# danshapero/sigma

Measured on AMD Instinct MI355X. Metric: SpMV GB/s (achieved HBM) + CG iters/sec on 5-pt Laplacian, N=1e7, higher is better.
Workload: dtype f64; 1 GPU; 5-point 2D Poisson CSR, 3162x3162 rows per GPU (rank 0: n=9998244, nnz=49978572), fp64 SpMV y=A*x; rows_per_gpu=9998244, nnz_per_gpu=49978572, parallelism=row-partition x1, matrix_resident_bytes_per_gpu=479920788, reference_layout_bytes_per_gpu=639735844, full=False

## Files before the change

### sigma_amd/__init__.py

```python
from __future__ import annotations

import ctypes as C
import os

import numpy as np

_HERE = os.path.dirname(os.path.abspath(__file__))
LIB_PATH = os.path.join(_HERE, "libsigma_hip.so")

SGM_HOST, SGM_DEVICE = 0, 1
FMT_CSR, FMT_ELL = 1, 2

_lib = None


class SigmaError(RuntimeError):

    def __init__(self, code, msg):
        super().__init__(f"[sigma_hip status {code}] {msg}")
        self.code = code


def build(force=False):
    import subprocess
# ... 221 lines not shown
        _ck(lib().sgm_graph_greedy_color_order(self._h, p.ctypes.data_as(C.c_void_p), ptrs.ctypes.data_as(C.c_void_p),
                                               C.c_int32(len(ptrs)), C.byref(nc)))
        return p, ptrs[:nc.value + 1].copy(), nc.value

    def left_permute(self, p):
        pp, w, _k = _arg(p, np.int32)
        _ck(lib().sgm_mat_left_permute(self._h, pp, C.c_int(w)))

    def right_permute(self, p):
        pp, w, _k = _arg(p, np.int32)
        _ck(lib().sgm_mat_right_permute(self._h, pp, C.c_int(w)))

    def set_option(self, name, value):
        if hasattr(self, "_build"):
            self._build()
        _ck(lib().sgm_mat_set_option(self._h, name.encode(), C.c_int(int(value))))
        return self

    @property
    def kernel(self):
        buf = C.create_string_buffer(64)
        _ck(lib().sgm_mat_kernel(self._h, buf, C.c_int(64)))
        return buf.value.decode()

    def set_solver(self, solver):
        self.solver = solver
        solver.setup(self)

    def set_preconditioner(self, pc):
        self.pc = pc
        pc.setup(self)

    def solve(self, x, b):
        if self.solver is None:
            raise SigmaError(1, "A%solve: no solver set (linear_operator_interface.f90:213-233)")
        return self.solver.solve(self, x, b, self.pc)

    def get(self, name, dtype):
        need = C.c_size_t(0)
        _ck(lib().sgm_mat_get(self._h, name.encode(), None, C.c_size_t(0), C.byref(need)))
        out = np.zeros(need.value // np.dtype(dtype).itemsize, dtype)
        _ck(lib().sgm_mat_get(self._h, name.encode(), C.c_void_p(out.ctypes.data), C.c_size_t(out.nbytes), None))
        return out

    def _triples(self, i, j, z=None):
        if not (_is_torch(i) or _is_torch(j) or (z is not None and _is_torch(z))):
# ... 971 lines not shown
```

### sigma_amd/csrc/sgm_internal.hpp

```cpp
#pragma once
#include <hip/hip_runtime.h>

#include <cstdarg>
#include <cstdint>
#include <cstdio>
#include <cstring>
#include <string>
#include <atomic>
#include <type_traits>
#include <utility>
#include <vector>

#include "../../include/sigma_hip.h"

namespace sgm {

extern std::string g_err;
int fail(int code, const char *fmt, ...);

#define SGM_HIP(call)                                                              \
    do {                                                                           \
        hipError_t e__ = (call);                                                   \
        if (e__ != hipSuccess)                                                     \
            return sgm::fail(SGM_ERR_HIP, "%s:%d: %s -> %s", __FILE__, __LINE__,   \
// ... 119 lines not shown
    int32_t recv_count = 0;
};

struct SliceSched { int32_t *tab = nullptr; int32_t lo = 0, hi = 0, grid = 0, iters = 0, band = 0; };

struct Part {
    MatOptions opt = g_opt.mat;
    int32_t n = 0;
    int32_t ncol_own = 0;
    int32_t n_halo = 0;
    int32_t int_lo = 0, int_hi = 0;
    int64_t nnz = 0;
    int64_t row_begin = 0;
    int32_t *rowptr = nullptr;
    int32_t *col = nullptr;
    double *val = nullptr;
    uint8_t *code = nullptr;
    int32_t *dict = nullptr;
    int32_t ndict = 0;
    int32_t dict_reach = 0;
    int32_t max_row = 0;
    double *sval = nullptr;
    uint32_t *scode = nullptr;
    int32_t *scol = nullptr;
    uint8_t *sbcode = nullptr;
    bool lean = false;
    double *sl_val = nullptr;
    int32_t *sl_col = nullptr;
    uint16_t *sl_perm = nullptr;
    int64_t *sl_off = nullptr;
    int64_t sl_total = 0;
    int32_t *sl_win0 = nullptr;
    int32_t sl_gs = 1;
    int32_t sl_span = 0;
    int32_t sw = 0;
    int32_t sched_period = 0;
    mutable SliceSched sched[3];
    mutable int nsched = 0;
    const int32_t *run_sched = nullptr;
    int32_t run_iters = 0;
    int32_t max_d = 0;
    int32_t *ecol = nullptr;
    double *eval = nullptr;
    int32_t *edeg = nullptr;
    uint8_t *ecode = nullptr;
    int32_t emdp = 0;
// ... 279 lines not shown
```

### sigma_amd/csrc/sgm_layouts.hip

```cpp
#include "sgm_spmv_select.hpp"

namespace sgm {

__global__ void k_dec1(int32_t *a, int64_t n)
{
    int64_t i = (int64_t)blockIdx.x * blockDim.x + threadIdx.x;
    const int64_t stride = (int64_t)gridDim.x * blockDim.x;
    for (; i < n; i += stride) a[i] -= 1;
}

__global__ void k_check_ptr1(const int32_t *__restrict__ ptr1, int64_t n, int64_t nnz, unsigned long long *bad)
{
    int64_t i = (int64_t)blockIdx.x * blockDim.x + threadIdx.x;
    const int64_t stride = (int64_t)gridDim.x * blockDim.x;
    for (; i <= n; i += stride) {
        const int32_t a = ptr1[i];
        bool ok = true;
        if (i == 0) ok = a == 1;
        if (i < n) ok = ok && ptr1[i + 1] >= a;
        else ok = ok && (int64_t)a - 1 == nnz;
        if (!ok) atomicMin(bad, (unsigned long long)i);
    }
}

// ... 144 lines not shown
    const int64_t nsl = ((int64_t)n + kSlRows - 1) / kSlRows;
    for (int64_t sl = blockIdx.x; sl < nsl; sl += gridDim.x)
        for (int r = threadIdx.x; r < kSlRows; r += blockDim.x) {
            const int64_t row = sl * kSlRows + r;
            int32_t k = 0, ke = 0;
            if (row < n) { k = rowptr[row]; ke = rowptr[row + 1]; }
            double *dst = sval + sl * (int64_t)W * kSlRows + r;
            for (int u = 0; u < W; ++u) dst[(int64_t)u * kSlRows] = k + u < ke ? val[k + u] : 0.0;
        }
}

__global__ __launch_bounds__(256) void k_sl_pack_ell(int32_t n, int32_t W, int32_t max_d, const double *__restrict__ eval,
                                                     double *__restrict__ sval)
{
    const int64_t nsl = ((int64_t)n + kSlRows - 1) / kSlRows;
    for (int64_t sl = blockIdx.x; sl < nsl; sl += gridDim.x)
        for (int r = threadIdx.x; r < kSlRows; r += blockDim.x) {
            const int64_t row = sl * kSlRows + r;
            double *dst = sval + sl * (int64_t)W * kSlRows + r;
            for (int u = 0; u < W; ++u) dst[(int64_t)u * kSlRows] = (row < n && u < max_d) ? eval[(int64_t)u * n + row] : 0.0;
        }
}

__global__ __launch_bounds__(256) void k_sl_unpack(int32_t n, int32_t W, const int32_t *__restrict__ rowptr, const uint32_t *__restrict__ scode,
                                                   const int32_t *__restrict__ dict, const double *__restrict__ sval,
                                                   int32_t *__restrict__ col, double *__restrict__ val, uint8_t *__restrict__ code)
{
    __shared__ int32_t dl[16];
    if (threadIdx.x < 16) dl[threadIdx.x] = dict[threadIdx.x];
    __syncthreads();
    for (int32_t i = blockIdx.x * blockDim.x + threadIdx.x; i < n; i += gridDim.x * blockDim.x) {
        const uint32_t cw = scode[i];
        int32_t k = rowptr[i];
        const double *src = sval + ((int64_t)(i >> 9) * W) * kSlRows + (i & (kSlRows - 1));
        for (int u = 0; u < W; ++u) {
            const uint32_t c = (cw >> (4 * u)) & 15u;
            if (c == 15u) break;
            if (col) col[k] = i + dl[c];
            if (val) val[k] = src[(int64_t)u * kSlRows];
            if (code) code[k] = (uint8_t)c;
            ++k;
        }
    }
}
__global__ __launch_bounds__(256) void k_sell_unpack(int32_t n, const int32_t *__restrict__ rowptr, const int64_t *__restrict__ off,
                                                     const uint16_t *__restrict__ perm, const int32_t *__restrict__ scol,
// ... 65 lines not shown
    (void)hipStreamSynchronize(g_rt.stream);
    dfree(p.val); dfree(p.col); dfree(p.code);
    p.val = nullptr; p.col = nullptr; p.code = nullptr;
}

int pack_sliced(Part &p)
{
    if (p.sl_val && p.n > 0) {
        const int64_t nch = (((int64_t)p.n + kSlRows - 1) / kSlRows) * (kSlRows / kSellChunk);
        hipLaunchKernelGGL(k_sell_fill, dim3((unsigned)std::min<int64_t>((nch + 3) / 4, 65536)), dim3(256), 0, g_rt.stream, p.n,
                           (const int32_t *)p.rowptr, (const int32_t *)nullptr, (const double *)p.val, (const int64_t *)p.sl_off,
                           (const uint16_t *)p.sl_perm, (int32_t *)nullptr, p.sl_val);
        SGM_HIP(hipGetLastError());
    }
    if ((!p.scode && !p.scol && !p.sbcode) || p.n == 0) return SGM_OK;
    const int64_t nsl = ((int64_t)p.n + kSlRows - 1) / kSlRows;
    if (p.ecol)
        hipLaunchKernelGGL(k_sl_pack_ell, dim3((unsigned)std::min<int64_t>(nsl, 65536)), dim3(256), 0, g_rt.stream, p.n, p.sw,
                           p.max_d, (const double *)p.eval, p.sval);
    else
        hipLaunchKernelGGL(k_sl_pack, dim3((unsigned)std::min<int64_t>(nsl, 65536)), dim3(256), 0, g_rt.stream, p.n, p.sw,
                           (const int32_t *)p.rowptr, (const double *)p.val, p.sval);
    SGM_HIP(hipGetLastError());
    return SGM_OK;
}

__global__ void k_fill32(int64_t n, int32_t *a, int32_t v)
{
    int64_t i = (int64_t)blockIdx.x * blockDim.x + threadIdx.x;
    const int64_t stride = (int64_t)gridDim.x * blockDim.x;
    for (; i < n; i += stride) a[i] = v;
}

constexpr int kDictSlots = 1024;
constexpr int32_t kDictEmpty = INT32_MIN;
__global__ __launch_bounds__(256) void k_dict_collect(int32_t n, const int32_t *__restrict__ rowptr, const int32_t *__restrict__ col,
                                                      int32_t *table, int *count, int *max_row)
{
    constexpr int kLocal = 512;
    __shared__ int32_t ltab[kLocal];
    __shared__ int lcount;
    for (int t = threadIdx.x; t < kLocal; t += 256) ltab[t] = kDictEmpty;
    if (threadIdx.x == 0) lcount = 0;
    __syncthreads();
    int mr = 0;
    int32_t mine[8];
#pragma unroll
// ... 465 lines not shown
    q.opt.csr_offset_dict = 0; q.opt.csr_sliced = 0; q.opt.csr_sell = 0; q.opt.csr_lean = 0; q.opt.slice_sched = 0;
    q.n = p.n; q.ncol_own = p.ncol_own; q.n_halo = 0; q.nnz = p.nnz; q.max_row = p.max_row;
    hipStream_t st = g_rt.stream;
    int rc = dalloc(&q.rowptr, (size_t)p.n + 1);
    if (rc == SGM_OK) rc = dalloc(&q.col, (size_t)p.nnz + 4);
    if (rc == SGM_OK) rc = dalloc(&q.val, (size_t)p.nnz + 2);
    if (rc != SGM_OK) { sgm_mat_destroy(C); return rc; }
    (void)hipMemcpyAsync(q.rowptr, p.rowptr, ((size_t)p.n + 1) * 4, hipMemcpyDeviceToDevice, st);
    (void)hipMemsetAsync(q.col + p.nnz, 0, 16, st);
    (void)hipMemsetAsync(q.val + p.nnz, 0, 16, st);
    if (p.nnz) {
        (void)hipMemcpyAsync(q.col, p.col, (size_t)p.nnz * 4, hipMemcpyDeviceToDevice, st);
        (void)hipMemcpyAsync(q.val, p.val, (size_t)p.nnz * 8, hipMemcpyDeviceToDevice, st);
    }
    if (hipStreamSynchronize(st) != hipSuccess || hipGetLastError() != hipSuccess) { sgm_mat_destroy(C); return fail(SGM_ERR_HIP, "clone_csr_plain: copy failed"); }
    *out = C;
    return SGM_OK;
}

int rebuild_csr_formats(Part &p)
{
    SGM_TRY(csr_need_arrays(p));
    p.lean = false;
    dfree(p.code); dfree(p.dict); dfree(p.sval); dfree(p.scode); dfree(p.scol); dfree(p.sbcode);
    p.code = nullptr; p.dict = nullptr; p.sval = nullptr; p.scode = nullptr; p.scol = nullptr; p.sbcode = nullptr;
    free_sell(p);
    free_ell_colblock(p);
    p.ndict = 0; p.dict_reach = 0; p.sw = 0; p.max_row = 0; p.sched_period = 0;
    free_slice_sched(p);
    return build_offset_dict(p, nullptr, nullptr);
}
int rebuild_ell_formats(Part &p)
{
    dfree(p.ecode); dfree(p.dict); dfree(p.sval); dfree(p.scode);
    p.ecode = nullptr; p.dict = nullptr; p.dict_reach = 0; p.emdp = 0; p.sval = nullptr; p.scode = nullptr; p.sw = 0; p.sched_period = 0;
    free_slice_sched(p);
    SGM_TRY(build_ell_offset_dict(p));
    SGM_TRY(build_ell_colblock(p));
    return refresh_ell_colblock_values(p);
}
int sgm_invalidate_transpose(sgm_mat A)
{
    if (A->T) { sgm_mat_destroy(A->T); A->T = nullptr; }
    dfree(A->tperm);
    A->tperm = nullptr;
    A->t_stale = true;
    return SGM_OK;
}

void free_part(Part &p)
{
    dfree(p.rowptr); dfree(p.col); dfree(p.val); dfree(p.code); dfree(p.dict); dfree(p.sval); dfree(p.scode); dfree(p.scol); dfree(p.sbcode); dfree(p.ecol); dfree(p.eval); dfree(p.edeg); dfree(p.ecode); dfree(p.xext);
    for (auto &nb : p.nbrs) { dfree(nb.send_idx); dfree(nb.send_buf); }
    free_slice_sched(p);
    free_ell_colblock(p);
    free_sell(p);
    p = Part();
}

}
```

### sigma_amd/csrc/sgm_mat.hip

```cpp
#include "sgm_spmv_select.hpp"
#include "sgm_krylov.hpp"

namespace sgm {

int stage_in(Staged &s, const double *v, int64_t n, int where, bool copy)
{
    if (where == SGM_DEVICE && (reinterpret_cast<uintptr_t>(v) & 15) == 0) {
        s.dev = const_cast<double *>(v);
        return SGM_OK;
    }
    SGM_TRY(dalloc(&s.dev, (size_t)n));
    s.owned = true;
    if (copy)
        SGM_HIP(hipMemcpyAsync(s.dev, v, (size_t)n * 8,
                               where == SGM_HOST ? hipMemcpyHostToDevice : hipMemcpyDeviceToDevice,
                               g_rt.stream));
    return SGM_OK;
}
int stage_out(const Staged &s, double *v, int64_t n, int where)
{
    if (!s.owned) return SGM_OK;
    SGM_HIP(hipMemcpyAsync(v, s.dev, (size_t)n * 8,
                           where == SGM_HOST ? hipMemcpyDeviceToHost : hipMemcpyDeviceToDevice,
                           g_rt.stream));
// ... 521 lines not shown
    A->parts.resize(1);
    A->parts[0].n = (int32_t)nloc_r;
    A->parts[0].ncol_own = (int32_t)nloc_c;
    int64_t g = (nloc_r + 4 * kBlock - 1) / (4 * kBlock);
    A->parts[0].dot_grid_override = (int)std::max<int64_t>(1, std::min<int64_t>(g, 2048));
    *out = A;
    return SGM_OK;
}

int sgm_mat_matvec_t(sgm_mat A, const double *x, double *y, int where)
{
    return matvec_t_impl(A, x, y, where, false);
}

int sgm_mat_matvec_t_add(sgm_mat A, const double *x, double *y, int where)
{
    return matvec_t_impl(A, x, y, where, true);
}

int sgm_mat_get(sgm_mat A, const char *name, void *out, size_t bytes, size_t *needed)
{
    SGM_TRY(require_init());
    if (!A || !name) return fail(SGM_ERR_BAD_ARG, "sgm_mat_get: null argument");
    if (A->distributed() || A->fmt == SGM_FMT_COMPOSITE)
        return fail(SGM_ERR_UNSUPPORTED, "sgm_mat_get: leaf single-GPU matrices only");
    const Part &p = A->parts[0];
    const std::string nm(name);
    std::vector<int32_t> vi;
    std::vector<double> vd;
    std::vector<int64_t> vq;
    const bool ell = A->fmt == SGM_FMT_ELL;
    if (!ell && (nm == "node" || nm == "val")) SGM_TRY(csr_need_arrays(p));
    struct Release { const Part &p; bool on; ~Release() { if (on) csr_release_arrays(p); } } rel{p, !ell};
    SGM_HIP(hipStreamSynchronize(g_rt.stream));
    if (!ell && nm == "ptr") {
        vi.resize((size_t)p.n + 1);
        SGM_HIP(hipMemcpy(vi.data(), p.rowptr, vi.size() * 4, hipMemcpyDeviceToHost));
        for (auto &v : vi) v += 1;
    } else if (!ell && nm == "node") {
        vi.resize((size_t)p.nnz);
        if (p.nnz) SGM_HIP(hipMemcpy(vi.data(), p.col, vi.size() * 4, hipMemcpyDeviceToHost));
        for (auto &v : vi) v += 1;
    } else if (!ell && nm == "val") {
        vd.resize((size_t)p.nnz);
        if (p.nnz) SGM_HIP(hipMemcpy(vd.data(), p.val, vd.size() * 8, hipMemcpyDeviceToHost));
    } else if (ell && nm == "max_d") {
// ... 68 lines not shown
extern "C" {

int sgm_mat_kernel(sgm_mat A, char *buf, int len)
{
    if (!A || !buf || len < 1) return fail(SGM_ERR_BAD_ARG, "sgm_mat_kernel: bad argument");
    char name[64];
    if (A->fmt == SGM_FMT_COMPOSITE) snprintf(name, sizeof name, "composite");
    else part_kernel_name(A->parts[0], A->fmt, name, sizeof name);
    snprintf(buf, (size_t)len, "%s", name);
    return SGM_OK;
}

static int64_t part_resident_bytes(const Part &p)
{
    int64_t b = 0;
    const int64_t nsl = ((int64_t)p.n + kSlRows - 1) / kSlRows;
    if (p.rowptr) b += 4 * ((int64_t)p.n + 1);
    if (p.col) b += 4 * (p.nnz + 4);
    if (p.val) b += 8 * (p.nnz + 2);
    if (p.code) b += p.nnz + 16;
    if (p.dict) b += 4 * 256;
    if (p.sval) b += 8 * nsl * kSlRows * p.sw;
    if (p.scode) b += 4 * nsl * kSlRows;
    if (p.scol) b += 4 * nsl * kSlRows * p.sw;
    if (p.sbcode) b += nsl * kSlRows * ((p.sw + 7) / 8 * 8);
    if (p.sl_val) b += 12 * p.sl_total + 2 * nsl * kSlRows + 8 * (nsl * (kSlRows / kSellChunk) + 1);
    if (p.ecol) b += 4 * (int64_t)p.n * p.max_d;
    if (p.eval) b += 8 * (int64_t)p.n * p.max_d;
    if (p.edeg) b += 4 * (int64_t)p.n;
    if (p.ecode) b += (int64_t)p.n * p.emdp;
    if (p.xext) b += 8 * p.xlen();
    b += ell_colblock_resident_bytes(p);
    for (const auto &nb : p.nbrs) b += (int64_t)nb.send_count * (nb.send_buf ? 12 : 4);
    return b;
}
static int64_t part_matvec_bytes(const sgm_mat_s *A, const Part &p)
{
    const int64_t nsl = ((int64_t)p.n + kSlRows - 1) / kSlRows;
    int64_t m;
    if (A->fmt == SGM_FMT_ELL) {
        if (use_ell_colblock(p)) return ell_colblock_matvec_bytes(p);
        if (use_sliced_ell(p)) m = nsl * kSlRows * (8 * (int64_t)p.sw + 4);
        else if (p.ecode && p.opt.ell_offset_dict) m = (int64_t)p.n * (8 * (int64_t)p.max_d + p.emdp);
        else m = 12 * (int64_t)p.n * p.max_d;
    } else if (use_ell_colblock(p)) return ell_colblock_matvec_bytes(p);
    else if (use_sliced(p)) m = nsl * kSlRows * (8 * (int64_t)p.sw + 4);
    else if (use_slicedb(p)) m = nsl * kSlRows * (8 * (int64_t)p.sw + (p.sw + 7) / 8 * 8);
    else if (use_sliced32(p)) m = nsl * kSlRows * 12 * (int64_t)p.sw;
    else if (use_sell(p)) {
        m = 12 * p.sl_total + 2 * nsl * kSlRows + 8 * nsl * (kSlRows / kSellChunk);
        if (p.sl_win0 && p.opt.csr_xwindow)
            return m + ((nsl + p.sl_gs - 1) / p.sl_gs) * (8 * (int64_t)p.sl_span + 4) + 8 * (int64_t)p.n;
    }
    else if (use_offset_dict(p)) m = 9 * p.nnz + 4 * ((int64_t)p.n + 1);
    else m = 12 * p.nnz + 4 * ((int64_t)p.n + 1);
    return m + 8 * p.xlen() + 8 * (int64_t)p.n;
}

int sgm_mat_footprint(sgm_mat A, int64_t *resident_bytes, int64_t *matvec_bytes)
{
    if (!A) return fail(SGM_ERR_BAD_ARG, "sgm_mat_footprint: null matrix");
    int64_t res = 0, mv = 0;
    if (A->fmt == SGM_FMT_COMPOSITE) {
        for (sgm_mat C : A->blocks) {
            if (!C) continue;
            int64_t r = 0, m = 0;
            SGM_TRY(sgm_mat_footprint(C, &r, &m));
            mv += m + 8 * (int64_t)C->nrow;
        }
// ... 23 lines not shown
```

### sigma_amd/csrc/sgm_runtime.hip

```cpp
#include "sgm_internal.hpp"

#include <algorithm>

namespace sgm {

std::string g_err;
Runtime g_rt;
Options g_opt;
Heartbeat g_hb;

int fail(int code, const char *fmt, ...)
{
    char buf[1024];
    va_list ap;
    va_start(ap, fmt);
    vsnprintf(buf, sizeof buf, fmt, ap);
    va_end(ap);
    g_err = buf;
    return code;
}

bool trace_on()
{
    static const bool on = getenv("SGM_TRACE") != nullptr;
// ... 69 lines not shown
    return nullptr;
}
int *solver_option_field(SolverOptions &o, const char *name)
{
    SGM_OPT(solver, cg_small) SGM_OPT(solver, bicgstab_small) SGM_OPT(solver, krylov_graph) SGM_OPT(solver, dot_order)
    SGM_OPT(solver, gmres_cgs2) SGM_OPT(solver, dist_halo_fused) SGM_OPT(solver, coop_spin_limit) SGM_OPT(solver, cg_coop_variant)
    SGM_OPT(solver, reorder_solve)
    return nullptr;
}
int *pc_option_field(PcOptions &o, const char *name)
{
    SGM_OPT(pc, ildu_strips) SGM_OPT(pc, ildu_rows) SGM_OPT(pc, pipeline_spin_limit) SGM_OPT(pc, ildu_reorder)
    return nullptr;
}
#undef SGM_OPT

int normalise_option(const char *name, int value, int *out)
{
    int v = value;
    if (!strcmp(name, "ell_colblock_cols")) v = std::min(kEllcbMaxCols, std::max(2, value)) & ~1;
    else if (!strcmp(name, "ell_colblock_rows")) v = value == 512 ? 512 : value == 256 ? 256 : 0;
    else if (!strcmp(name, "ildu_reorder")) v = value != 0;
    else if (!strcmp(name, "csr_sell")) v = value < 0 ? 0 : value > 2 ? 2 : value;
    else if (!strcmp(name, "csr_lean") || !strcmp(name, "csr_xwindow")) v = value != 0;
    else if (!strcmp(name, "slice_sched")) v = value <= 0 ? 0 : value == 1 ? 1 : std::max(4, value);
    else if (!strcmp(name, "krylov_graph")) v = value <= 0 ? 0 : value == 1 ? 1 : std::max(16, (value + 15) / 16 * 16);
    else if (!strcmp(name, "cg_small")) v = std::max(0, value);
    else if (!strcmp(name, "dist_halo_fused") || !strcmp(name, "reorder_solve")) v = value < 0 ? 0 : value > 2 ? 2 : value;
    else if (!strcmp(name, "coop_spin_limit")) v = std::max(0, value);
    else if (!strcmp(name, "gmres_cgs2")) v = value != 0;
    else if (!strcmp(name, "cg_coop_variant")) {
        const int r = value & 15;
        if (value < 0 || value > 31 || (r != 0 && r != 1 && r != 2 && r != 4 && r != 8))
            return fail(SGM_ERR_BAD_ARG, "option cg_coop_variant: rows per thread 0 (by size), 1, 2, 4 or 8, + 16 = no one-XCD variant");
    }
    else if (!strcmp(name, "coloring_pass")) v = value < 0 ? 0 : value > 2 ? 2 : value;
    else if (!strcmp(name, "pipeline_spin_limit")) v = std::max(0, value);
    else if (!strcmp(name, "dot_order") && value != 0 && value != 1)
        return fail(SGM_ERR_BAD_ARG, "option dot_order is 0 (tree) or 1 (the reference's sequential order)");
    *out = v;
    return SGM_OK;
}

}

using namespace sgm;
// ... 120 lines not shown
```

### sigma_amd/csrc/sgm_spmv.hip

```cpp
#include "sgm_spmv_device.hpp"
#include "sgm_plan_host.hpp"

#include <cassert>

namespace sgm {


template <int BLOCK, int VPT, bool NT, bool ADD, bool DOT_W, bool DOT_YY>
__global__ __launch_bounds__(BLOCK) void k_csr_spmv(
    int32_t n, const int32_t *__restrict__ rowptr, const int32_t *__restrict__ col,
    const double *__restrict__ val, const double *__restrict__ x, double *__restrict__ y,
    const double *__restrict__ w, double *__restrict__ part_wy, double *__restrict__ part_yy,
    const int *__restrict__ flag_done, int gen, int remap)
{
    constexpr int TILE = 2 * BLOCK * VPT;
    __shared__ double prod[TILE];
    __shared__ double red[BLOCK / 64];
    if (stopped(flag_done, gen)) return;

    const int tid = threadIdx.x;
    const bool chain = (remap & kChainBit) != 0;
    const int64_t nrb = ((int64_t)n + BLOCK - 1) / BLOCK;
    double dwy = 0.0, dyy = 0.0;

// ... 290 lines not shown
                double xv[U], vv[U];
#pragma unroll
                for (int u = 0; u < U; ++u)
                    if (u < cnt) {
                        const int o = k + u - ts;
                        xv[u] = CW == 1 ? x[row + dl[cl[o]]] : x[(int32_t)cl4[o]];
                        vv[u] = vl[o];
                    }
#pragma unroll
                for (int u = 0; u < U; ++u)
                    if (u < cnt) z = z + vv[u] * xv[u];
                k += cnt;
            }
        }
        if (row < n) {
            const double yi = row_value<ADD>(y0, z, chain);
            __builtin_nontemporal_store(yi, y + row);
            dots_add<DOT_W, DOT_YY>(DOT_W ? w[row] : 0.0, yi, dwy, dyy);
        }
    }
    dots_write<BLOCK, DOT_W, DOT_YY>(dwy, dyy, red, part_wy, part_yy);
}

template <int W, bool ADD, bool DOT_W, bool DOT_YY>
__global__ __launch_bounds__(256) void k_csr_sl(
    int32_t n, const uint32_t *__restrict__ scode, const int32_t *__restrict__ dict,
    const double *__restrict__ sval, const double *__restrict__ x, double *__restrict__ y,
    const double *__restrict__ w, double *__restrict__ part_wy, double *__restrict__ part_yy,
    const int *__restrict__ flag_done, int gen, int remap, const int32_t *__restrict__ sched, int sched_iters)
{
    constexpr int BLOCK = 256;
    __shared__ int32_t dl[16];
    __shared__ double red[BLOCK / 64];
    const int st = stop_flag(flag_done);
    const int tid = threadIdx.x;
    const bool chain = (remap & kChainBit) != 0;
    const int32_t dv = tid < 16 ? dict[tid] : 0;
    const int64_t nsl = ((int64_t)n + kSlRows - 1) / kSlRows;
    double dwy = 0.0, dyy = 0.0;

    const int64_t first = first_slice(remap & kSliceMapBits);
    int64_t sl = sched ? sched[blockIdx.x] : first;
    int sit = 0;
    u32x2 cw = {0xffffffffu, 0xffffffffu};
    f64x2 v[W];
    auto load_slice = [&](int64_t s_) {
        const int32_t row_ = (int32_t)(s_ * kSlRows) + 2 * tid;
        cw = __builtin_nontemporal_load(reinterpret_cast<const u32x2 *>(scode + row_));
        const f64x2 *vb = reinterpret_cast<const f64x2 *>(sval + s_ * (int64_t)(W * kSlRows)) + tid;
#pragma unroll
        for (int u = 0; u < W; ++u) v[u] = __builtin_nontemporal_load(vb + u * BLOCK);
    };
    bool have = sl >= 0 && sl < nsl;
    if (have) load_slice(sl);
    if (stop_hit(st, gen)) return;
    if (tid < 16) dl[tid] = dv;
    __syncthreads();
    while (have) {
        int64_t nxt = sl + gridDim.x;
        if (sched) { ++sit; nxt = sit < sched_iters ? sched[(int64_t)sit * gridDim.x + blockIdx.x] : -1; }
        const int32_t row = (int32_t)(sl * kSlRows) + 2 * tid;
        const f64x2 y0 = pair_load_y0<ADD>(y, row, n);
        const f64x2 z = sl_row_sums<W>(pair_start<ADD>(y0, chain), cw, v, x, row, dl);
        pair_finish<ADD, DOT_W, DOT_YY>(y, w, row, n, y0, z, chain, dwy, dyy);
        sl = nxt;
        have = sl >= 0 && sl < nsl;
        if (have) load_slice(sl);
    }
    dots_write<BLOCK, DOT_W, DOT_YY>(dwy, dyy, red, part_wy, part_yy);
}

template <bool ADD, bool DOT_W, bool DOT_YY, bool XW = false, int GS = 1>
__global__ __launch_bounds__(256 * GS) void k_csr_sell(
    int32_t n, const int64_t *__restrict__ off, const uint16_t *__restrict__ perm, const int32_t *__restrict__ scol,
    const double *__restrict__ sval, const double *__restrict__ x, double *__restrict__ y, const double *__restrict__ w,
    double *__restrict__ part_wy, double *__restrict__ part_yy, const int *__restrict__ flag_done, int gen, int remap,
    const int32_t *__restrict__ win0 = nullptr, int32_t span = 0, int32_t xlen = 0)
{
    constexpr int BLOCK = 256 * GS;
    extern __shared__ double xs[];
    __shared__ double red[BLOCK / 64];
    const int st = stop_flag(flag_done);
    const int lane = threadIdx.x & 63;
    const int wave = __builtin_amdgcn_readfirstlane(threadIdx.x >> 6);
    const bool chain = (remap & kChainBit) != 0;
    const int64_t nsl = ((int64_t)n + kSlRows - 1) / kSlRows;
    double dwy = 0.0, dyy = 0.0;
    if (stop_hit(st, gen)) return;

    int64_t first = blockIdx.x;
// ... 286 lines not shown
#define LV(T)                                                                                                               \
    if (tile == T) {                                                                                                        \
        if (!dict)                                                                                                          \
            hipLaunchKernelGGL((k_csr_do<kSpmvBlock, T, 4, F::add, F::dot_w, F::dot_yy>), dim3(grid), dim3(kSpmvBlock), 0, g_rt.stream, p.n, \
                               p.rowptr, reinterpret_cast<const uint8_t *>(p.col), p.dict, p.val, a.x, a.y, a.w, a.pwy, a.pyy, \
                               a.flag, a.gen, chain_bit(a));                                                                \
        else if constexpr (T <= kDoMaxCodeTile)                                                                             \
            hipLaunchKernelGGL((k_csr_do<kSpmvBlock, T, 1, F::add, F::dot_w, F::dot_yy>), dim3(grid), dim3(kSpmvBlock), 0, g_rt.stream, p.n, \
                               p.rowptr, p.code, p.dict, p.val, a.x, a.y, a.w, a.pwy, a.pyy, a.flag, a.gen, chain_bit(a));  \
        return;                                                                                                             \
    }
        SGM_DO_TILES(LV)
#undef LV
    });
}

static void launch_csr_sl(const Part &p, int grid, const SpmvArgs &a)
{
    const int remap = slice_map_mode(grid, p.n) | chain_bit(a);
    with_flags(a, [&](auto flags) {
        using F = decltype(flags);
#define LV(WW)                                                                                                              \
    if (p.sw == WW) {                                                                                                       \
        hipLaunchKernelGGL((k_csr_sl<WW, F::add, F::dot_w, F::dot_yy>), dim3(grid), dim3(256), 0, g_rt.stream, p.n, p.scode, p.dict, p.sval, \
                           a.x, a.y, a.w, a.pwy, a.pyy, a.flag, a.gen, remap, p.run_sched, p.run_iters);                    \
        return;                                                                                                             \
    }
        SGM_SL_WIDTHS(LV)
#undef LV
    });
}

static void launch_csr_sl32(const Part &p, int grid, const SpmvArgs &a)
{
    const int remap = slice_map_mode(grid, p.n) | chain_bit(a);
    with_flags(a, [&](auto flags) {
        using F = decltype(flags);
#define LV(WW)                                                                                                              \
    if (p.sw == WW) {                                                                                                       \
        hipLaunchKernelGGL((k_csr_sl32<WW, F::add, F::dot_w, F::dot_yy>), dim3(grid), dim3(256), 0, g_rt.stream, p.n, p.scol, p.sval, a.x, a.y, \
                           a.w, a.pwy, a.pyy, a.flag, a.gen, remap);                                                        \
        return;                                                                                                             \
    }
        SGM_SL32_WIDTHS(LV)
#undef LV
    });
}

// ... 43 lines not shown
static_assert(kEllGrid <= kMaxGrid, "one partial slot per workgroup");
int ell_grid(const Part &p)
{
    if (use_ell_colblock(p)) return ell_colblock_grid(p);
    if (use_sliced_ell(p)) {
        const int64_t nsl = ((int64_t)p.n + kSlRows - 1) / kSlRows;
        return (int)std::max<int64_t>(1, std::min<int64_t>(nsl, nsl >= 32768 ? kMaxGrid : kMaxGrid / 2));
    }
    int64_t g = ((int64_t)p.n + kBlock - 1) / kBlock;
    int64_t cap = kEllGrid;
    if (p.ecode && p.opt.ell_offset_dict && p.emdp == 16) cap = std::min<int64_t>(cap, (int64_t)5 * g_rt.num_cu);
    return (int)std::max<int64_t>(1, std::min<int64_t>(g, cap));
}

static void launch_ell(const Part &p, int grid, const SpmvArgs &a)
{
    if (use_ell_colblock(p)) {
        (void)launch_ell_colblock(p, grid, a);
        return;
    }
    if (use_sliced_ell(p)) {
        Part v;
        v.n = p.n; v.scode = p.scode; v.dict = p.dict; v.sval = p.sval; v.sw = p.sw;
        if (const SliceSched *ss = slice_sched(p, 0, p.n, grid)) { v.run_sched = ss->tab; v.run_iters = ss->iters; }
        launch_csr_sl(v, grid, a);
        return;
    }
    with_flags(a, [&](auto flags) {
        using F = decltype(flags);
        if (p.ecode && p.opt.ell_offset_dict) {
#define LD(M)                                                                                                               \
    hipLaunchKernelGGL((k_ell_do<M, F::add, F::dot_w, F::dot_yy>), dim3(grid), dim3(kBlock), 0, g_rt.stream, p.n, p.max_d, p.ecode, p.dict, \
                       p.eval, a.x, a.y, a.w, a.pwy, a.pyy, a.flag, a.gen, chain_bit(a))
            if (p.emdp == 4) LD(4);
            else if (p.emdp == 8) LD(8);
            else LD(16);
#undef LD
            return;
        }
        hipLaunchKernelGGL((k_ell_spmv<kEllU, true, F::add, F::dot_w, F::dot_yy>), dim3(grid), dim3(kBlock), 0, g_rt.stream, p.n, p.max_d, p.ecol,
                           p.eval, a.x, a.y, a.w, a.pwy, a.pyy, a.flag, a.gen, chain_bit(a));
    });
}

int resident_per_cu(bool row_owner, int tile, int cw)
{
// ... 43 lines not shown
    if (dalloc(&d, tab.size()) != SGM_OK) return nullptr;
    if (hipMemcpy(d, tab.data(), tab.size() * sizeof(int32_t), hipMemcpyHostToDevice) != hipSuccess) { dfree(d); return nullptr; }
    ss.tab = d; ss.iters = iters;
    return &ss;
}
void free_slice_sched(Part &p)
{
    for (int i = 0; i < p.nsched; ++i) { dfree(p.sched[i].tab); p.sched[i] = SliceSched(); }
    p.nsched = 0;
}

static void launch_range(const Part &p, const RowRange &r, const SpmvArgs &a)
{
    Part v;
    v.opt = p.opt;
    v.n = r.hi - r.lo;
    v.nnz = (int64_t)((double)p.nnz * v.n / (p.n > 0 ? p.n : 1));
    v.n_halo = p.n_halo; v.ncol_own = p.ncol_own;
    v.rowptr = p.rowptr + r.lo; v.col = p.col; v.val = p.val; v.code = p.code; v.dict = p.dict;
    v.max_row = p.max_row;
    const bool sliced = use_sliced(p), slicedb = !sliced && use_slicedb(p), sliced32 = !sliced && !slicedb && use_sliced32(p);
    if (sliced || slicedb)
        if (const SliceSched *ss = slice_sched(p, r.lo, r.hi, r.grid)) { v.run_sched = ss->tab; v.run_iters = ss->iters; }
    if (sliced) { v.sval = p.sval + (int64_t)r.lo * p.sw; v.scode = p.scode + r.lo; v.sw = p.sw; }
    if (slicedb) { v.sval = p.sval + (int64_t)r.lo * p.sw; v.sbcode = p.sbcode + (int64_t)r.lo * ((p.sw + 7) / 8 * 8); v.sw = p.sw; }
    if (sliced32) { v.sval = p.sval + (int64_t)r.lo * p.sw; v.scol = p.scol + (int64_t)r.lo * p.sw; v.sw = p.sw; }
    const bool sell = !sliced && !slicedb && !sliced32 && use_sell(p);
    if (sell) {
        v.sl_val = p.sl_val; v.sl_col = p.sl_col;
        v.sl_off = p.sl_off + r.lo / kSellChunk; v.sl_perm = p.sl_perm + r.lo;
        v.sl_gs = p.sl_gs;
        v.sl_win0 = p.sl_win0 ? p.sl_win0 + r.lo / (kSlRows * p.sl_gs) : nullptr; v.sl_span = p.sl_span;
    }
    const bool dict = use_offset_dict(p);
    SpmvArgs ar = a;
    ar.y = a.y + r.lo;
    ar.w = a.w ? a.w + r.lo : nullptr;
    ar.pwy = a.pwy ? a.pwy + r.part_off : nullptr;
    ar.pyy = a.pyy ? a.pyy + r.part_off : nullptr;
    if (dict && !sliced32 && !sell) ar.x = a.x + r.lo;
    if (sliced) launch_csr_sl(v, r.grid, ar);
    else if (slicedb) launch_csr_slb(v, r.grid, ar);
    else if (sliced32) launch_csr_sl32(v, r.grid, ar);
    else if (sell) launch_csr_sell(v, r.grid, ar);
    else if (use_row_owner(p)) launch_csr_do(v, r.grid, ar);
    else if (use_row_lines(p)) launch_csr_rl(v, r.grid, ar);
    else launch_csr(v, r.grid, ar);
// ... 148 lines not shown
```

### sigma_amd/csrc/sgm_spmv_device.hpp

```cpp
#pragma once
#include "sgm_spmv_select.hpp"

namespace sgm {

__device__ __forceinline__ int stop_flag(const int *__restrict__ flag_done) { return flag_done ? *flag_done : 0; }
__device__ __forceinline__ bool stop_hit(int st, int gen) { return st && gen >= st; }
__device__ __forceinline__ bool stopped(const int *__restrict__ flag_done, int gen)
{
    if (flag_done) {
        const int st = *flag_done;
        if (stop_hit(st, gen)) return true;
    }
    return false;
}

__device__ __forceinline__ int64_t rowblock_of(int it, int b, int grid)
{
    const int per = grid >> 3;
    return (int64_t)it * grid + (int64_t)(b & 7) * per + (b >> 3);
}

__device__ __forceinline__ int64_t first_slice(int mode)
{
    if (!mode) return blockIdx.x;
// ... 58 lines not shown
        __builtin_nontemporal_store(yi.x, y + row);
        dots_add<DOT_W, DOT_YY>(DOT_W ? w[row] : 0.0, yi.x, dwy, dyy);
    }
}

template <int W>
__device__ __forceinline__ f64x2 sl_row_sums(f64x2 z, u32x2 cw, const f64x2 (&v)[W], const double *__restrict__ x, int32_t row,
                                             const int32_t *dl)
{
    double xa[W], xb[W];
#pragma unroll
    for (int u = 0; u < W; ++u) {
        const uint32_t ca = (cw.x >> (4 * u)) & 15u, cb = (cw.y >> (4 * u)) & 15u;
        xa[u] = ca != 15u ? x[row + dl[ca]] : 0.0;
        xb[u] = cb != 15u ? x[row + 1 + dl[cb]] : 0.0;
    }
#pragma unroll
    for (int u = 0; u < W; ++u) {
        if (((cw.x >> (4 * u)) & 15u) != 15u) z.x = z.x + v[u].x * xa[u];
        if (((cw.y >> (4 * u)) & 15u) != 15u) z.y = z.y + v[u].y * xb[u];
    }
    return z;
}

template <int W>
__device__ __forceinline__ f64x2 slb_row_sums(f64x2 z, const double *__restrict__ sval, const uint8_t *__restrict__ sbcode, int64_t sl, int tid,
                                              const double *__restrict__ x, int32_t row, const int32_t *dl)
{
    constexpr int BLOCK = kSlRows / 2;
    constexpr int NCH = (W + 7) / 8;
    const f64x2 *vb = reinterpret_cast<const f64x2 *>(sval + sl * (int64_t)W * kSlRows) + tid;
    const u32x4s *cb = reinterpret_cast<const u32x4s *>(sbcode + sl * (int64_t)(NCH * 8 * kSlRows)) + tid;
    auto chunk = [&](int c, auto cnt_tag) {
        constexpr int CNT = decltype(cnt_tag)::value;
        f64x2 v[CNT];
        double xa[CNT], xb[CNT];
        const u32x4s cw = __builtin_nontemporal_load(cb + c * BLOCK);
#pragma unroll
        for (int u = 0; u < CNT; ++u) v[u] = __builtin_nontemporal_load(vb + (c * 8 + u) * BLOCK);
#pragma unroll
        for (int u = 0; u < CNT; ++u) {
            const uint32_t ca = ((u < 4 ? cw.x : cw.y) >> (8 * (u & 3))) & 255u;
            const uint32_t cbv = ((u < 4 ? cw.z : cw.w) >> (8 * (u & 3))) & 255u;
            xa[u] = ca != 255u ? x[row + dl[ca]] : 0.0;
            xb[u] = cbv != 255u ? x[row + 1 + dl[cbv]] : 0.0;
        }
// ... 21 lines not shown
```

### sigma_amd/csrc/sgm_spmv_select.hpp

```cpp
#pragma once
#include "sgm_internal.hpp"

#include <type_traits>

#include <hipcub/hipcub.hpp>

#include <algorithm>
#include <cstdlib>
#include <string>
#include <vector>

namespace sgm {

typedef double f64x2 __attribute__((ext_vector_type(2)));
typedef int i32x2 __attribute__((ext_vector_type(2)));
typedef int i32x4 __attribute__((ext_vector_type(4)));
typedef uint32_t u32x2 __attribute__((ext_vector_type(2)));
typedef uint16_t u16x2 __attribute__((ext_vector_type(2)));
typedef unsigned int u32x4s __attribute__((ext_vector_type(4)));
#define SGM_SLB_WIDTHS(X) X(9) X(12) X(15) X(16) X(19) X(20) X(24) X(25) X(27) X(28) X(32)
#define SGM_SL_WIDTHS(X) X(3) X(5) X(7) X(8)
#define SGM_SL32_WIDTHS(X) X(3) X(5) X(7) X(8) X(12) X(16) X(20) X(24) X(28) X(32)
constexpr int kSlRows = 512;
constexpr int kSellChunk = 128;
// ... 35 lines not shown
        else f(SpmvFlags<false, false, false>{});
    }
}

int resident_per_cu(bool row_owner, int tile, int cw);
static const SliceSched *slice_sched(const Part &p, int32_t lo, int32_t hi, int grid);
void free_slice_sched(Part &p);
int ell_grid(const Part &p);
bool use_ell_colblock(const Part &p);
int ell_colblock_grid(const Part &p);
int build_ell_colblock(Part &p);
int refresh_ell_colblock_values(Part &p);
void free_ell_colblock(Part &p);
int launch_ell_colblock(const Part &p, int grid, const SpmvArgs &a);
int64_t ell_colblock_resident_bytes(const Part &p);
int64_t ell_colblock_matvec_bytes(const Part &p);
static bool use_offset_dict(const Part &p) { return (p.code || (p.lean && p.dict)) && p.opt.csr_offset_dict; }
static bool use_sliced(const Part &p) { return p.scode && p.opt.csr_sliced && p.opt.csr_offset_dict; }
static bool use_sliced32(const Part &p) { return p.scol && p.opt.csr_sliced && !p.ecol; }
static bool use_slicedb(const Part &p) { return p.sbcode && p.opt.csr_sliced && p.opt.csr_offset_dict; }
static bool use_sell(const Part &p) { return p.sl_val && p.opt.csr_sliced && p.opt.csr_sell && !p.ecol; }
static bool any_sliced(const Part &p) { return use_sliced(p) || use_sliced32(p) || use_slicedb(p) || use_sell(p); }
static bool use_sliced_ell(const Part &p) { return p.ecol && p.scode && p.opt.csr_sliced && p.opt.ell_offset_dict; }
static bool use_row_owner(const Part &p)
{
    return use_offset_dict(p) || (p.opt.csr_row_owner && p.max_row > 0 && p.max_row <= 64);
}

static bool use_row_lines(const Part &p)
{
    return p.opt.csr_row_lines && !any_sliced(p) && !use_row_owner(p) && p.n > 0 && p.max_row <= 4096 &&
           p.nnz >= 16 * (int64_t)p.n && (int64_t)p.max_row * p.n <= 4 * p.nnz;
}
int row_lines_resident_per_cu();

#define SGM_DO_TILES(X) X(1024) X(1536) X(1920) X(2048) X(4096)
constexpr int kDoMaxCodeTile = 2048;
static int do_tile_for(const Part &p)
{
    static const int tiles[] = {1024, 1536, 1920, 2048, 4096};
    const int nt = use_offset_dict(p) ? 4 : 5;
    const double per_block = (double)p.nnz / (p.n > 0 ? p.n : 1) * kSpmvBlock + 4;
    for (int i = 0; i < nt; ++i)
        if (per_block <= tiles[i]) return tiles[i];
    return tiles[nt - 1];
}
// ... 51 lines not shown
```

Before: 6344 GB/s.

## Replace per-entry sliced values with a per-offset value table when uniform

At pack time, two kernel passes check whether every nonzero sharing the same dictionary offset code has the same value. If so, a 16-entry value table is stored and a templated sliced SpMV kernel reads coefficients from shared memory instead of streaming sval. For constant-coefficient stencils this removes most of the matrix value traffic, leaving the code words plus x and y. The cost is extra setup kernels and a host sync. The bytes reported per matvec also shrink, so the achieved-GB/s figure may not track the speedup.

Result: slower. 4523 GB/s (-28.7%).

```diff
diff --git a/sigma_amd/__init__.py b/sigma_amd/__init__.py
--- a/sigma_amd/__init__.py
+++ b/sigma_amd/__init__.py
@@ -267,6 +267,13 @@
         buf = C.create_string_buffer(64)
         _ck(lib().sgm_mat_kernel(self._h, buf, C.c_int(64)))
         return buf.value.decode()
+
+    @property
+    def value_table(self):
+        if hasattr(self, "_build"):
+            self._build()
+        got = self.get("value_table", np.int32)
+        return bool(got[0]) if got.size == 1 else [bool(v) for v in got]
 
     def set_solver(self, solver):
         self.solver = solver
diff --git a/sigma_amd/csrc/sgm_internal.hpp b/sigma_amd/csrc/sgm_internal.hpp
--- a/sigma_amd/csrc/sgm_internal.hpp
+++ b/sigma_amd/csrc/sgm_internal.hpp
@@ -165,6 +165,8 @@
     int32_t max_row = 0;
     double *sval = nullptr;
     uint32_t *scode = nullptr;
+    uint64_t *vtab = nullptr;
+    bool vtab_ok = false;
     int32_t *scol = nullptr;
     uint8_t *sbcode = nullptr;
     bool lean = false;
diff --git a/sigma_amd/csrc/sgm_layouts.hip b/sigma_amd/csrc/sgm_layouts.hip
--- a/sigma_amd/csrc/sgm_layouts.hip
+++ b/sigma_amd/csrc/sgm_layouts.hip
@@ -190,6 +190,60 @@
         }
 }
 
+template <bool CHECK>
+__global__ __launch_bounds__(256) void k_vtab_pass(int32_t n, int32_t W, const uint32_t *__restrict__ scode, const double *__restrict__ sval,
+                                                   uint64_t *vtab)
+{
+    __shared__ uint64_t lt[16];
+    __shared__ int lset[16];
+    __shared__ int bad;
+    const int tid = threadIdx.x;
+    if (tid < 16) { lt[tid] = CHECK ? vtab[tid] : 0; lset[tid] = 0; }
+    if (tid == 0) bad = 0;
+    __syncthreads();
+    const int64_t nsl = ((int64_t)n + kSlRows - 1) / kSlRows;
+    bool mismatch = false;
+    for (int64_t sl = blockIdx.x; sl < nsl; sl += gridDim.x)
+        for (int r = tid; r < kSlRows; r += 256) {
+            const uint32_t cw = scode[sl * kSlRows + r];
+            const uint64_t *src = reinterpret_cast<const uint64_t *>(sval) + sl * (int64_t)W * kSlRows + r;
+            for (int u = 0; u < W; ++u) {
+                const uint32_t c = (cw >> (4 * u)) & 15u;
+                if (c == 15u) continue;
+                const uint64_t bits = src[(int64_t)u * kSlRows];
+                if (CHECK) mismatch = mismatch || bits != lt[c];
+                else if (!lset[c] || lt[c] != bits) { lt[c] = bits; lset[c] = 1; }
+            }
+        }
+    if (CHECK) {
+        if (mismatch) bad = 1;
+        __syncthreads();
+        if (tid == 0 && bad) vtab[15] = 0;
+    } else {
+        __syncthreads();
+        if (tid < 15 && lset[tid] && *(volatile uint64_t *)(vtab + tid) != lt[tid]) vtab[tid] = lt[tid];
+        if (tid == 15 && blockIdx.x == 0) vtab[15] = 1;
+    }
+}
+static int value_table_check(Part &p)
+{
+    p.vtab_ok = false;
+    if (!p.scode || !p.dict || !p.sval || p.sw > 8 || p.n == 0) return SGM_OK;
+    hipStream_t st = g_rt.stream;
+    if (!p.vtab) SGM_TRY(dalloc(&p.vtab, (size_t)16));
+    SGM_HIP(hipMemsetAsync(p.vtab, 0, 16 * sizeof(uint64_t), st));
+    const int64_t nsl = ((int64_t)p.n + kSlRows - 1) / kSlRows;
+    const unsigned grid = (unsigned)std::min<int64_t>(nsl, 2048);
+    hipLaunchKernelGGL(k_vtab_pass<false>, dim3(grid), dim3(256), 0, st, p.n, p.sw, (const uint32_t *)p.scode, (const double *)p.sval, p.vtab);
+    hipLaunchKernelGGL(k_vtab_pass<true>, dim3(grid), dim3(256), 0, st, p.n, p.sw, (const uint32_t *)p.scode, (const double *)p.sval, p.vtab);
+    SGM_HIP(hipGetLastError());
+    uint64_t ok = 0;
+    SGM_HIP(hipMemcpyAsync(&ok, p.vtab + 15, sizeof ok, hipMemcpyDeviceToHost, st));
+    SGM_HIP(hipStreamSynchronize(st));
+    p.vtab_ok = ok == 1;
+    return SGM_OK;
+}
+
 __global__ __launch_bounds__(256) void k_sl_unpack(int32_t n, int32_t W, const int32_t *__restrict__ rowptr, const uint32_t *__restrict__ scode,
                                                    const int32_t *__restrict__ dict, const double *__restrict__ sval,
                                                    int32_t *__restrict__ col, double *__restrict__ val, uint8_t *__restrict__ code)
@@ -301,7 +355,7 @@
         hipLaunchKernelGGL(k_sl_pack, dim3((unsigned)std::min<int64_t>(nsl, 65536)), dim3(256), 0, g_rt.stream, p.n, p.sw,
                            (const int32_t *)p.rowptr, (const double *)p.val, p.sval);
     SGM_HIP(hipGetLastError());
-    return SGM_OK;
+    return value_table_check(p);
 }
 
 __global__ void k_fill32(int64_t n, int32_t *a, int32_t v)
@@ -813,8 +867,9 @@
 {
     SGM_TRY(csr_need_arrays(p));
     p.lean = false;
-    dfree(p.code); dfree(p.dict); dfree(p.sval); dfree(p.scode); dfree(p.scol); dfree(p.sbcode);
+    dfree(p.code); dfree(p.dict); dfree(p.sval); dfree(p.scode); dfree(p.scol); dfree(p.sbcode); dfree(p.vtab);
     p.code = nullptr; p.dict = nullptr; p.sval = nullptr; p.scode = nullptr; p.scol = nullptr; p.sbcode = nullptr;
+    p.vtab = nullptr; p.vtab_ok = false;
     free_sell(p);
     free_ell_colblock(p);
     p.ndict = 0; p.dict_reach = 0; p.sw = 0; p.max_row = 0; p.sched_period = 0;
@@ -823,8 +878,9 @@
 }
 int rebuild_ell_formats(Part &p)
 {
-    dfree(p.ecode); dfree(p.dict); dfree(p.sval); dfree(p.scode);
+    dfree(p.ecode); dfree(p.dict); dfree(p.sval); dfree(p.scode); dfree(p.vtab);
     p.ecode = nullptr; p.dict = nullptr; p.dict_reach = 0; p.emdp = 0; p.sval = nullptr; p.scode = nullptr; p.sw = 0; p.sched_period = 0;
+    p.vtab = nullptr; p.vtab_ok = false;
     free_slice_sched(p);
     SGM_TRY(build_ell_offset_dict(p));
     SGM_TRY(build_ell_colblock(p));
@@ -841,7 +897,7 @@
 
 void free_part(Part &p)
 {
-    dfree(p.rowptr); dfree(p.col); dfree(p.val); dfree(p.code); dfree(p.dict); dfree(p.sval); dfree(p.scode); dfree(p.scol); dfree(p.sbcode); dfree(p.ecol); dfree(p.eval); dfree(p.edeg); dfree(p.ecode); dfree(p.xext);
+    dfree(p.rowptr); dfree(p.col); dfree(p.val); dfree(p.code); dfree(p.dict); dfree(p.sval); dfree(p.scode); dfree(p.vtab); dfree(p.scol); dfree(p.sbcode); dfree(p.ecol); dfree(p.eval); dfree(p.edeg); dfree(p.ecode); dfree(p.xext);
     for (auto &nb : p.nbrs) { dfree(nb.send_idx); dfree(nb.send_buf); }
     free_slice_sched(p);
     free_ell_colblock(p);
diff --git a/sigma_amd/csrc/sgm_mat.hip b/sigma_amd/csrc/sgm_mat.hip
--- a/sigma_amd/csrc/sgm_mat.hip
+++ b/sigma_amd/csrc/sgm_mat.hip
@@ -567,6 +567,15 @@
 {
     SGM_TRY(require_init());
     if (!A || !name) return fail(SGM_ERR_BAD_ARG, "sgm_mat_get: null argument");
+    if (!strcmp(name, "value_table") && A->fmt != SGM_FMT_COMPOSITE) {
+        const size_t sz = A->parts.size() * sizeof(int32_t);
+        if (needed) *needed = sz;
+        if (out && sz) {
+            if (bytes < sz) return fail(SGM_ERR_BAD_ARG, "sgm_mat_get: buffer too small (%zu < %zu)", bytes, sz);
+            for (size_t i = 0; i < A->parts.size(); ++i) static_cast<int32_t *>(out)[i] = use_value_table(A->parts[i]) ? 1 : 0;
+        }
+        return SGM_OK;
+    }
     if (A->distributed() || A->fmt == SGM_FMT_COMPOSITE)
         return fail(SGM_ERR_UNSUPPORTED, "sgm_mat_get: leaf single-GPU matrices only");
     const Part &p = A->parts[0];
@@ -681,6 +690,7 @@
     if (p.dict) b += 4 * 256;
     if (p.sval) b += 8 * nsl * kSlRows * p.sw;
     if (p.scode) b += 4 * nsl * kSlRows;
+    if (p.vtab) b += 16 * 8;
     if (p.scol) b += 4 * nsl * kSlRows * p.sw;
     if (p.sbcode) b += nsl * kSlRows * ((p.sw + 7) / 8 * 8);
     if (p.sl_val) b += 12 * p.sl_total + 2 * nsl * kSlRows + 8 * (nsl * (kSlRows / kSellChunk) + 1);
@@ -696,14 +706,15 @@
 static int64_t part_matvec_bytes(const sgm_mat_s *A, const Part &p)
 {
     const int64_t nsl = ((int64_t)p.n + kSlRows - 1) / kSlRows;
+    const int64_t sl_tab = nsl * kSlRows * 4 + 16 * 8;
     int64_t m;
     if (A->fmt == SGM_FMT_ELL) {
         if (use_ell_colblock(p)) return ell_colblock_matvec_bytes(p);
-        if (use_sliced_ell(p)) m = nsl * kSlRows * (8 * (int64_t)p.sw + 4);
+        if (use_sliced_ell(p)) m = use_value_table(p) ? sl_tab : nsl * kSlRows * (8 * (int64_t)p.sw + 4);
         else if (p.ecode && p.opt.ell_offset_dict) m = (int64_t)p.n * (8 * (int64_t)p.max_d + p.emdp);
         else m = 12 * (int64_t)p.n * p.max_d;
     } else if (use_ell_colblock(p)) return ell_colblock_matvec_bytes(p);
-    else if (use_sliced(p)) m = nsl * kSlRows * (8 * (int64_t)p.sw + 4);
+    else if (use_sliced(p)) m = use_value_table(p) ? sl_tab : nsl * kSlRows * (8 * (int64_t)p.sw + 4);
     else if (use_slicedb(p)) m = nsl * kSlRows * (8 * (int64_t)p.sw + (p.sw + 7) / 8 * 8);
     else if (use_sliced32(p)) m = nsl * kSlRows * 12 * (int64_t)p.sw;
     else if (use_sell(p)) {
diff --git a/sigma_amd/csrc/sgm_runtime.hip b/sigma_amd/csrc/sgm_runtime.hip
--- a/sigma_amd/csrc/sgm_runtime.hip
+++ b/sigma_amd/csrc/sgm_runtime.hip
@@ -115,6 +115,7 @@
     else if (!strcmp(name, "ell_colblock_rows")) v = value == 512 ? 512 : value == 256 ? 256 : 0;
     else if (!strcmp(name, "ildu_reorder")) v = value != 0;
     else if (!strcmp(name, "csr_sell")) v = value < 0 ? 0 : value > 2 ? 2 : value;
+    else if (!strcmp(name, "csr_sliced")) v = value < 0 ? 0 : value > 3 ? 3 : value;
     else if (!strcmp(name, "csr_lean") || !strcmp(name, "csr_xwindow")) v = value != 0;
     else if (!strcmp(name, "slice_sched")) v = value <= 0 ? 0 : value == 1 ? 1 : std::max(4, value);
     else if (!strcmp(name, "krylov_graph")) v = value <= 0 ? 0 : value == 1 ? 1 : std::max(16, (value + 15) / 16 * 16);
diff --git a/sigma_amd/csrc/sgm_spmv.hip b/sigma_amd/csrc/sgm_spmv.hip
--- a/sigma_amd/csrc/sgm_spmv.hip
+++ b/sigma_amd/csrc/sgm_spmv.hip
@@ -336,20 +336,24 @@
     dots_write<BLOCK, DOT_W, DOT_YY>(dwy, dyy, red, part_wy, part_yy);
 }
 
-template <int W, bool ADD, bool DOT_W, bool DOT_YY>
+template <int W, bool ADD, bool DOT_W, bool DOT_YY, bool TAB = false>
 __global__ __launch_bounds__(256) void k_csr_sl(
     int32_t n, const uint32_t *__restrict__ scode, const int32_t *__restrict__ dict,
     const double *__restrict__ sval, const double *__restrict__ x, double *__restrict__ y,
     const double *__restrict__ w, double *__restrict__ part_wy, double *__restrict__ part_yy,
-    const int *__restrict__ flag_done, int gen, int remap, const int32_t *__restrict__ sched, int sched_iters)
+    const int *__restrict__ flag_done, int gen, int remap, const int32_t *__restrict__ sched, int sched_iters,
+    const double *__restrict__ vtab = nullptr)
 {
     constexpr int BLOCK = 256;
     __shared__ int32_t dl[16];
+    __shared__ double vt[TAB ? 16 : 1];
     __shared__ double red[BLOCK / 64];
     const int st = stop_flag(flag_done);
     const int tid = threadIdx.x;
     const bool chain = (remap & kChainBit) != 0;
     const int32_t dv = tid < 16 ? dict[tid] : 0;
+    double tv = 0.0;
+    if (TAB) tv = tid < 16 ? vtab[tid] : 0.0;
     const int64_t nsl = ((int64_t)n + kSlRows - 1) / kSlRows;
     double dwy = 0.0, dyy = 0.0;
 
@@ -357,29 +361,41 @@
     int64_t sl = sched ? sched[blockIdx.x] : first;
     int sit = 0;
     u32x2 cw = {0xffffffffu, 0xffffffffu};
-    f64x2 v[W];
+    f64x2 v[TAB ? 1 : W];
     auto load_slice = [&](int64_t s_) {
         const int32_t row_ = (int32_t)(s_ * kSlRows) + 2 * tid;
         cw = __builtin_nontemporal_load(reinterpret_cast<const u32x2 *>(scode + row_));
-        const f64x2 *vb = reinterpret_cast<const f64x2 *>(sval + s_ * (int64_t)(W * kSlRows)) + tid;
-#pragma unroll
-        for (int u = 0; u < W; ++u) v[u] = __builtin_nontemporal_load(vb + u * BLOCK);
+        if constexpr (!TAB) {
+            const f64x2 *vb = reinterpret_cast<const f64x2 *>(sval + s_ * (int64_t)(W * kSlRows)) + tid;
+#pragma unroll
+            for (int u = 0; u < W; ++u) v[u] = __builtin_nontemporal_load(vb + u * BLOCK);
+        }
     };
     bool have = sl >= 0 && sl < nsl;
     if (have) load_slice(sl);
     if (stop_hit(st, gen)) return;
     if (tid < 16) dl[tid] = dv;
+    if (TAB && tid < 16) vt[tid] = tv;
     __syncthreads();
     while (have) {
         int64_t nxt = sl + gridDim.x;
         if (sched) { ++sit; nxt = sit < sched_iters ? sched[(int64_t)sit * gridDim.x + blockIdx.x] : -1; }
         const int32_t row = (int32_t)(sl * kSlRows) + 2 * tid;
         const f64x2 y0 = pair_load_y0<ADD>(y, row, n);
-        const f64x2 z = sl_row_sums<W>(pair_start<ADD>(y0, chain), cw, v, x, row, dl);
-        pair_finish<ADD, DOT_W, DOT_YY>(y, w, row, n, y0, z, chain, dwy, dyy);
-        sl = nxt;
-        have = sl >= 0 && sl < nsl;
-        if (have) load_slice(sl);
+        if constexpr (TAB) {
+            const u32x2 cwc = cw;
+            sl = nxt;
+            have = sl >= 0 && sl < nsl;
+            if (have) load_slice(sl);
+            const f64x2 z = sl_row_sums_tab<W>(pair_start<ADD>(y0, chain), cwc, vt, x, row, dl);
+            pair_finish<ADD, DOT_W, DOT_YY>(y, w, row, n, y0, z, chain, dwy, dyy);
+        } else {
+            const f64x2 z = sl_row_sums<W>(pair_start<ADD>(y0, chain), cw, v, x, row, dl);
+            pair_finish<ADD, DOT_W, DOT_YY>(y, w, row, n, y0, z, chain, dwy, dyy);
+            sl = nxt;
+            have = sl >= 0 && sl < nsl;
+            if (have) load_slice(sl);
+        }
     }
     dots_write<BLOCK, DOT_W, DOT_YY>(dwy, dyy, red, part_wy, part_yy);
 }
@@ -712,8 +728,13 @@
         using F = decltype(flags);
 #define LV(WW)                                                                                                              \
     if (p.sw == WW) {                                                                                                       \
-        hipLaunchKernelGGL((k_csr_sl<WW, F::add, F::dot_w, F::dot_yy>), dim3(grid), dim3(256), 0, g_rt.stream, p.n, p.scode, p.dict, p.sval, \
-                           a.x, a.y, a.w, a.pwy, a.pyy, a.flag, a.gen, remap, p.run_sched, p.run_iters);                    \
+        if (p.vtab_ok)                                                                                                      \
+            hipLaunchKernelGGL((k_csr_sl<WW, F::add, F::dot_w, F::dot_yy, true>), dim3(grid), dim3(256), 0, g_rt.stream, p.n, p.scode, p.dict, \
+                               (const double *)nullptr, a.x, a.y, a.w, a.pwy, a.pyy, a.flag, a.gen, remap, p.run_sched, p.run_iters, \
+                               reinterpret_cast<const double *>(p.vtab));                                                   \
+        else                                                                                                                \
+            hipLaunchKernelGGL((k_csr_sl<WW, F::add, F::dot_w, F::dot_yy>), dim3(grid), dim3(256), 0, g_rt.stream, p.n, p.scode, p.dict, p.sval, \
+                               a.x, a.y, a.w, a.pwy, a.pyy, a.flag, a.gen, remap, p.run_sched, p.run_iters, (const double *)nullptr); \
         return;                                                                                                             \
     }
         SGM_SL_WIDTHS(LV)
@@ -803,6 +824,7 @@
     if (use_sliced_ell(p)) {
         Part v;
         v.n = p.n; v.scode = p.scode; v.dict = p.dict; v.sval = p.sval; v.sw = p.sw;
+        v.vtab = p.vtab; v.vtab_ok = use_value_table(p);
         if (const SliceSched *ss = slice_sched(p, 0, p.n, grid)) { v.run_sched = ss->tab; v.run_iters = ss->iters; }
         launch_csr_sl(v, grid, a);
         return;
@@ -892,7 +914,10 @@
     const bool sliced = use_sliced(p), slicedb = !sliced && use_slicedb(p), sliced32 = !sliced && !slicedb && use_sliced32(p);
     if (sliced || slicedb)
         if (const SliceSched *ss = slice_sched(p, r.lo, r.hi, r.grid)) { v.run_sched = ss->tab; v.run_iters = ss->iters; }
-    if (sliced) { v.sval = p.sval + (int64_t)r.lo * p.sw; v.scode = p.scode + r.lo; v.sw = p.sw; }
+    if (sliced) {
+        v.sval = p.sval + (int64_t)r.lo * p.sw; v.scode = p.scode + r.lo; v.sw = p.sw;
+        v.vtab = p.vtab; v.vtab_ok = use_value_table(p);
+    }
     if (slicedb) { v.sval = p.sval + (int64_t)r.lo * p.sw; v.sbcode = p.sbcode + (int64_t)r.lo * ((p.sw + 7) / 8 * 8); v.sw = p.sw; }
     if (sliced32) { v.sval = p.sval + (int64_t)r.lo * p.sw; v.scol = p.scol + (int64_t)r.lo * p.sw; v.sw = p.sw; }
     const bool sell = !sliced && !slicedb && !sliced32 && use_sell(p);
diff --git a/sigma_amd/csrc/sgm_spmv_device.hpp b/sigma_amd/csrc/sgm_spmv_device.hpp
--- a/sigma_amd/csrc/sgm_spmv_device.hpp
+++ b/sigma_amd/csrc/sgm_spmv_device.hpp
@@ -104,6 +104,32 @@
     }
     return z;
 }
+template <int W>
+__device__ __forceinline__ f64x2 sl_row_sums_tab(f64x2 z, u32x2 cw, const double *vt, const double *__restrict__ x, int32_t row,
+                                                 const int32_t *dl)
+{
+    typedef double f64x2u __attribute__((ext_vector_type(2), aligned(8)));
+    double xa[W], xb[W];
+#pragma unroll
+    for (int u = 0; u < W; ++u) {
+        const uint32_t ca = (cw.x >> (4 * u)) & 15u, cb = (cw.y >> (4 * u)) & 15u;
+        if (ca == cb) {
+            f64x2 p = {0.0, 0.0};
+            if (ca != 15u) p = *reinterpret_cast<const f64x2u *>(x + row + dl[ca]);
+            xa[u] = p.x; xb[u] = p.y;
+        } else {
+            xa[u] = ca != 15u ? x[row + dl[ca]] : 0.0;
+            xb[u] = cb != 15u ? x[row + 1 + dl[cb]] : 0.0;
+        }
+    }
+#pragma unroll
+    for (int u = 0; u < W; ++u) {
+        const uint32_t ca = (cw.x >> (4 * u)) & 15u, cb = (cw.y >> (4 * u)) & 15u;
+        if (ca != 15u) z.x = z.x + vt[ca] * xa[u];
+        if (cb != 15u) z.y = z.y + vt[cb] * xb[u];
+    }
+    return z;
+}
 
 template <int W>
 __device__ __forceinline__ f64x2 slb_row_sums(f64x2 z, const double *__restrict__ sval, const uint8_t *__restrict__ sbcode, int64_t sl, int tid,
diff --git a/sigma_amd/csrc/sgm_spmv_select.hpp b/sigma_amd/csrc/sgm_spmv_select.hpp
--- a/sigma_amd/csrc/sgm_spmv_select.hpp
+++ b/sigma_amd/csrc/sgm_spmv_select.hpp
@@ -81,6 +81,12 @@
 static bool use_sell(const Part &p) { return p.sl_val && p.opt.csr_sliced && p.opt.csr_sell && !p.ecol; }
 static bool any_sliced(const Part &p) { return use_sliced(p) || use_sliced32(p) || use_slicedb(p) || use_sell(p); }
 static bool use_sliced_ell(const Part &p) { return p.ecol && p.scode && p.opt.csr_sliced && p.opt.ell_offset_dict; }
+constexpr int32_t kValueTableMinRows = 1 << 21;
+static bool use_value_table(const Part &p)
+{
+    if (!p.vtab || !p.vtab_ok || !(p.ecol ? use_sliced_ell(p) : use_sliced(p))) return false;
+    return p.opt.csr_sliced == 2 || (p.opt.csr_sliced == 1 && p.n >= kValueTableMinRows);
+}
 static bool use_row_owner(const Part &p)
 {
     return use_offset_dict(p) || (p.opt.csr_row_owner && p.max_row > 0 && p.max_row <= 64);
```
